# DefaultRui/VLN-VER

Hardware: AMD Instinct MI355X
Metric: viewpoints/sec (multi-view->voxel fwd+bwd), vocc.py config (higher is better)
Workload: dtype bf16

## Files before the change

include/ver_ops.h:

```cpp
#ifndef VER_OPS_H
#define VER_OPS_H

#include <stdint.h>

#ifdef __cplusplus
extern "C" {
#endif

#define VER_ABI_VERSION 31

#define VER_OK            0
#define VER_EINVAL       -1
#define VER_EUNSUPPORTED -2
#define VER_ELAUNCH      -3

#define VER_F32  0
#define VER_BF16 1

#define VER_I32  0
#define VER_I64  1

int         ver_abi_version(void);
const char* ver_last_error(void);

// ... 130 lines not shown
int ver_run_gather(const void* image, long image_stride, const int32_t* run_start, const int32_t* aug_idx,
                   void* rows, int B, int n_rows, int runs, int run_len, int n_aug, int row_elems, int dtype,
                   void* stream);
int ver_run_scatter(const void* rows, void* image, long image_stride, const int32_t* run_start, int B,
                    int n_rows, int runs, int run_len, int row_elems, int dtype, void* stream);

#define VER_OCC_MLP_CENTERED 2
long ver_occ_mlp_image_bytes(void);
int ver_occ_mlp_vector_floats(void);
int ver_occ_mlp_pack(const float* W1, const float* W2, const float* W3, void* image, void* stream);
int ver_occ_mlp_forward(const void* x, const void* image, const float* vectors, void* logits,
                        long N, int width, int classes, float eps, int flags, void* stream);
int ver_occ_mlp_forward_stats(const void* x, const void* image, const float* vectors, void* logits, float* rstd,
                              long N, int width, int classes, float eps, int flags, void* stream);
int ver_occ_mlp_backward(const void* x, const void* grad_logits, const void* image, const float* vectors,
                         void* grad_x, void* grad_a1, void* grad_a2, void* h1,
                         float* param_grads, long N, int width, int classes, float eps, int first_linear,
                         void* stream);
int ver_occ_mlp_backward_fused(const void* x, const void* grad_logits, const float* W2, const float* W3,
                               const float* vectors, void* grad_x, float* param_grads, long N, int width,
                               int classes, float eps, const float* grad_scale, int flags, void* stream);
int ver_occ_mlp_backward_fused_stats(const void* x, const void* grad_logits, const float* W2, const float* W3,
                                     const float* vectors, const float* rstd, void* grad_x, float* param_grads, long N,
                                     int width, int classes, float eps, const float* grad_scale, int flags, void* stream);
long ver_occ_mlp_backward_fused_slab_bytes(long N);
int ver_occ_mlp_backward_fused_slabs(const void* x, const void* grad_logits, const float* W2, const float* W3,
                                     const float* vectors, const float* rstd, void* grad_x, float* param_grads, float* slabs,
                                     long slab_bytes, long N, int width, int classes, float eps, const float* grad_scale,
                                     int flags, void* stream);

long ver_occ_predict_blocks(long N);
int  ver_occ_predict(const void* logits, int dtype, long N, int C, float threshold, int32_t* block_work,
                     int64_t* pairs, int64_t* count, void* stream);

int  ver_occ_confusion(const void* logits, int dtype, long rows_per_sample, int samples, int C, const uint8_t* labels,
                       const float* thresholds, int num_thresholds, int64_t* hist, void* stream);

int ver_occ_mlp_confusion(const void* x, const void* image, const float* vectors, const uint8_t* labels,
                          long rows_per_sample, int samples, const float* thresholds, int num_thresholds,
                          int64_t* hist, int width, int classes, float eps, int flags, void* stream);
int ver_occ_mlp_classes(const void* x, const void* image, const float* vectors, uint8_t* cls, float* prob,
                        long N, float threshold, int width, int classes, float eps, int flags, void* stream);

int  ver_wgrad_tn_splits(long M, int Ka, int N);
int  ver_wgrad_tn_splits_ld(long M, int Ka, int N, long ld);
long ver_wgrad_tn_workspace(long M, int Ka, int N, int splits);
int  ver_wgrad_tn(const void* a, long lda, const void* g, long ldg, long M, int Ka, int N, void* out, long ldo,
                  int out_dtype, int splits, int flags, void* workspace, long workspace_bytes, void* stream);
int  ver_wgrad_tn_segments(const void* lattice, int layout, int B, int H, int W, int C, const int* taps, int nseg, const void* cst,
                           int ncst, int cw, const void* g, long ldg, int N, void* out, long ldo, int out_dtype, int splits,
                           void* workspace, long workspace_bytes, void* stream);
int  ver_wgrad_tn_segments_splits(int B, int H, int W, long Ka, int N, long ldg);

int  ver_gemm_nn(const void* a, long lda, const void* w, long ldw, const float* bias, void* c, long ldc, long M, int K,
                 int N, int flags, void* stream);
int  ver_gemm_nn_taps(const void* lattice, int layout, int B, int H, int W, int C, const int* taps, int ntaps, const void* w,
                      long ldw, const float* rowpos, const float* bias, void* c, long ldc, int N, void* stream);
int  ver_gemm_nn_segments(const void* lattice, int layout, int B, int H, int W, int C, const int* taps, int ntaps,
                          const void* cst, int ncst, int cw, const void* w, long ldw, const float* rowpos, const float* bias,
                          void* c, long ldc, int N, void* stream);
int  ver_gemm_nn_planes(const void* lattice, int layout, int B, int H, int W, int C, long plane_elems, int nplanes,
                        const int* tap_plane, const int* taps, int ntaps, const void* cst, int ncst, int cw, const void* w,
                        long ldw, const float* rowpos, const float* bias, void* c, long ldc, int N, void* stream);
int  ver_gemm_nn_splits(long M, int K, int N);
int  ver_gemm_nn_splitk(const void* a, long lda, const void* w, long ldw, const float* bias, void* c, long ldc, long M, int K,
                        int N, int splits, void* workspace, long workspace_bytes, void* stream);

int ver_clip_adamw_step(void* const* table, const long* sizes, const int* chunk_tensor, const int* chunk_index,
                        int n_tensors, int n_chunks, int chunk_elems, float* partial, float* norm_out, float max_norm,
                        float lr, float beta1, float beta2, float eps, float weight_decay, long step, void* stream);

int ver_clip_adamw_step_tensors(void* const* table, const long* sizes, const int* chunk_tensor, const int* chunk_index,
                                const float* hyper, int* steps, int n_tensors, int n_chunks, int chunk_elems, float* partial,
                                float* norm_out, float max_norm, void* stream);

int ver_grad_pack(const void* const* table, const long* sizes, const long* offsets, const int* chunk_tensor,
                  const int* chunk_index, int n_tensors, int n_chunks, int chunk_elems, float scale, void* flat,
                  int flat_dtype, void* stream);

int ver_clip_adamw_step_flat(void* const* table, const long* sizes, const long* offsets, const int* chunk_tensor,
                             const int* chunk_index, const float* hyper, int* steps, const void* flat, int flat_dtype,
                             int n_tensors, int n_chunks, int chunk_elems, float* partial, float* norm_out, float max_norm,
                             void* stream);

int ver_lsa_solve(const float* cost, const int32_t* ncols, int32_t* match, int32_t* bad,
                  int P, int R, int Ccap, void* stream);

int ver_box3d_overlaps(const float* a, const int32_t* na, const float* b, const int32_t* nb, float* iou,
                       int S, int Acap, int Bcap, void* stream);

int ver_det_match(const float* pred_boxes, const int32_t* pred_labels, const float* pred_scores,
                  const uint8_t* pred_valid, const float* gt_boxes, const int32_t* gt_labels, const int32_t* ngt,
                  const float* thresholds, int num_thresholds, float* iou_max, int32_t* gt_index,
                  uint8_t* tp_bits, int64_t* npos, int num_classes, int S, int Pcap, int Gcap, void* stream);

int ver_det_costs(const void* cls, int cls_dtype, const float* box, int box_ld, const float* gt,
                  const int64_t* gt_labels, const int32_t* counts, float* cost, int L, int B, int Q, int C, int Gcap,
                  float w_cls, float alpha, float gamma, float eps, float w_reg, void* stream);
int ver_det_set_loss_forward(const void* cls, int cls_dtype, const float* box, int box_ld, const int32_t* match,
                             const float* gt, const int64_t* gt_labels, const int32_t* counts,
                             const float* code_weights, float* sums, int32_t* npos, int32_t* bad, int L, int B, int Q,
                             int C, int Gcap, float alpha, float gamma, void* stream);
int ver_det_set_loss_backward(const void* cls, int cls_dtype, const float* box, int box_ld, const int32_t* match,
                              const float* gt, const int64_t* gt_labels, const int32_t* counts,
                              const float* code_weights, const float* scale, void* grad_cls, float* grad_box, int L,
                              int B, int Q, int C, int Gcap, float alpha, float gamma, void* stream);
// ... 33 lines not shown
```

scratch/prof_summary.py:

```python
import sqlite3, sys, collections
def kernel_stats(path, out):
    db = sqlite3.connect(path); cur = db.cursor()
    rows = cur.execute("select name, count(*), sum(end-start), avg(end-start), min(end-start), max(end-start) from kernels group by name order by 3 desc").fetchall()
    tot = sum(r[2] for r in rows)
    with open(out, 'w') as f:
        f.write('# rocprofv3 --kernel-trace --stats summary (from %s)\n' % path.split('/')[-1])
        f.write('Name,Calls,TotalDurationNs,AverageNs,Percentage,MinNs,MaxNs\n')
        for r in rows:
            f.write('"%s",%d,%d,%.1f,%.2f,%d,%d\n' % (r[0].replace('"', "'")[:160], r[1], r[2], r[3], 100.0 * r[2] / tot, r[4], r[5]))
def pmc_stats(path, out, like=('k_sca', 'k_project', 'k_build', 'k_zero', 'k_msda', 'k_lattice', 'k_occ_mlp', 'k_focal')):
    db = sqlite3.connect(path); cur = db.cursor()
    rows = cur.execute("select kernel_name, counter_name, sum(value), count(distinct dispatch_id) from counters_collection group by kernel_name, counter_name").fetchall()
    with open(out, 'a') as f:
        f.write('# rocprofv3 --pmc per-dispatch averages (from %s)\n' % path.split('/')[-1])
        f.write('Kernel,Counter,PerDispatch,Dispatches\n')
        for k, c, v, n in sorted(rows):
            if any(l in k for l in like):
                f.write('"%s",%s,%.1f,%d\n' % (k.replace('(anonymous namespace)::', '').split('(')[0][:80], c, v / n, n))
def kernel_stats_timed(path, out, total_steps, skip_steps):
    db = sqlite3.connect(path); cur = db.cursor()
    rows = cur.execute("select name, start, end from kernels order by start").fetchall()
    per = collections.OrderedDict()
    for n, s, e in rows:
        per.setdefault(n, []).append(e - s)
    stats = []
    for n, d in per.items():
        c = len(d)
        if c % total_steps == 0 and c >= total_steps:
            k = c // total_steps
            d = d[skip_steps * k:]
            steps = total_steps - skip_steps
        else:
            steps = 0
        stats.append((n, len(d), sum(d), sum(d) / len(d), min(d), max(d), steps))
    stats.sort(key=lambda r: -r[2])
    tot = sum(r[2] for r in stats if r[6]) or 1
    with open(out, 'w') as f:
        f.write('# rocprofv3 --kernel-trace, dispatches of the TIMED steps only (%d of %d steps; from %s)\n' % (total_steps - skip_steps, total_steps, path.split('/')[-1]))
        f.write('Name,Calls,TotalDurationNs,AverageNs,PercentageOfTimedSteps,MinNs,MaxNs,Steps,NsPerStep\n')
        for n, c, t, a, lo, hi, st in stats:
            f.write('"%s",%d,%d,%.1f,%.2f,%d,%d,%d,%.0f\n' % (n.replace('"', "'")[:160], c, t, a, 100.0 * t / tot if st else 0.0, lo, hi, st, t / st if st else 0))
if __name__ == '__main__':
    if sys.argv[1] == 'kernels_timed':
        kernel_stats_timed(sys.argv[2], sys.argv[3], int(sys.argv[4]), int(sys.argv[5])); sys.exit(0)
    mode, path, out = sys.argv[1:4]
    (kernel_stats if mode == 'kernels' else pmc_stats)(path, out)
```

vln-ver_amd/csrc/build.py:

```python
import os
import subprocess
import sys
import tempfile

HERE = os.path.dirname(os.path.abspath(__file__))
PKG = os.path.dirname(HERE)
LIB = os.path.join(PKG, 'libver_hip.so')
SOURCES = ['ver_abi.hip', 'ver_msda.hip', 'ver_sca.hip', 'ver_lattice.hip', 'ver_mlp.hip', 'ver_loss.hip', 'ver_occ_mlp.hip', 'ver_layout.hip', 'ver_addln.hip', 'ver_post.hip', 'ver_wgrad.hip', 'ver_gemm.hip', 'ver_optim.hip', 'ver_assign.hip', 'ver_boxiou.hip', 'ver_setloss.hip', 'ver_decode.hip', 'ver_targets.hip', 'ver_dattn3d.hip', 'ver_mha.hip']
HEADERS = ['ver_common.h', 'ver_classify.h', 'ver_gemm_tile.h', os.path.join('..', '..', 'include', 'ver_ops.h')]
FLAGS = ['-O3', '-std=c++17', '--offload-arch=gfx950', '-fPIC', '-shared', '-munsafe-fp-atomics',
         '-Wall', '-Wno-unused-function']


TARGET_FEATURES = {'ver_occ_mlp.hip': ['-packed-fp32-ops']}
_HOST_PASS_NOISE = 'is not a recognized feature for this target'

OBJ_DIR = os.path.join(HERE, 'build')
CFLAGS = [f for f in FLAGS if f != '-shared']


def _newer(target, deps):
    if not os.path.exists(target):
        return True
    t = os.path.getmtime(target)
    return any(os.path.getmtime(d) > t for d in deps)


def stale():
    deps = [os.path.join(HERE, f) for f in SOURCES + HEADERS] + [os.path.abspath(__file__)]
    return _newer(LIB, deps)


ASAN_LIB = os.path.join(PKG, 'libver_hip_asan.so')
ASAN_FLAGS = ['-O1', '-g', '-fsanitize=address', '-fno-gpu-sanitize', '-shared-libsan', '-fno-omit-frame-pointer']


def asan_runtime():
    import glob
    hits = sorted(glob.glob('/opt/rocm/lib/llvm/lib/clang/*/lib/linux/libclang_rt.asan-x86_64.so'))
    return hits[-1] if hits else None


def build_hip(force=False, verbose=True, defines=(), lib=None, asan=False):
    if asan:
        lib = lib or ASAN_LIB
    lib = lib or LIB
    if not force and not defines and lib == LIB and not stale():
        return LIB
    if asan and not force and not _newer(lib, [os.path.join(HERE, f) for f in SOURCES + HEADERS] + [os.path.abspath(__file__)]):
        return lib
    hipcc = os.environ.get('HIPCC', '/opt/rocm/bin/hipcc')
    tag = ''.join('_' + d.replace('=', '-') for d in defines)
    os.makedirs(OBJ_DIR, exist_ok=True)
    hdrs = [os.path.join(HERE, h) for h in HEADERS] + [os.path.abspath(__file__)]
    objs, procs = [], []
    for src in SOURCES:
        path = os.path.join(HERE, src)
        mytag = tag if (defines and any(d.split('=')[0] in open(path).read() for d in defines)) else ''
        if asan:
            mytag += '_asan'
        obj = os.path.join(OBJ_DIR, src.replace('.hip', mytag + '.o'))
# ... 29 lines not shown
```

vln-ver_amd/csrc/ver_layout.hip:

```cpp
#include "ver_common.h"

namespace {
__device__ __forceinline__ uint16_t f32_to_bf16(float f) {
    const uint32_t u = __float_as_uint(f);
    if ((u & 0x7fffffffu) > 0x7f800000u) return (uint16_t)((u >> 16) | 0x40u);
    return (uint16_t)((u + 0x7fffu + ((u >> 16) & 1u)) >> 16);
}
constexpr int kTaps = 75;
constexpr int kPairs = 64;
}
#define VER_BLOCKS_VEC_SLICES 8

template <bool BF16>
__global__ __launch_bounds__(256) void k_convt_weight_fwd(const float* __restrict__ w, void* __restrict__ k, long P) {
    __shared__ float tile[kPairs * kTaps + 1];
    const long p0 = (long)blockIdx.x * kPairs;
    const int np = (int)((P - p0) < kPairs ? (P - p0) : kPairs);
    for (int i = threadIdx.x; i < np * kTaps; i += 256) tile[i] = w[p0 * kTaps + i];
    __syncthreads();
    for (int i = threadIdx.x; i < kTaps * kPairs; i += 256) {
        const int t = i / kPairs, p = i % kPairs;
        if (p >= np) continue;
        const int a = t / 25, b = (t / 5) % 5, c = t % 5;
        const float v = tile[p * kTaps + ((2 - a) * 5 + (4 - b)) * 5 + (4 - c)];
// ... 378 lines not shown
    }
}
__device__ __forceinline__ long row_map_piece(const RowMapLds& t, int period, int c, int piece_off) {
    const int4 ch = t.ch[c];
    int off = ch.z + piece_off, row = ch.y;
    while (off >= period) off -= period, ++row;
    const int sg = t.slot_seg[off >> 2];
    const int4 sp = t.seg[sg];
    return t.seg_base[sg] + (long)row * sp.z + ch.x * sp.y + (off - sp.x);
}
}

template <int LAYOUT, bool TO_ROWS, int CH>
__global__ __launch_bounds__(256) void k_lattice_rows(uint16_t* __restrict__ cl, uint16_t* __restrict__ rows, RowMap map,
                                                      int B, int Z, int H, int W, int C, int R) {
    extern __shared__ __attribute__((aligned(16))) unsigned char smem[];
    constexpr int VC = 8, VX = 4;
    const int P = R * W;
    const int ncb = (C + CH - 1) / CH;
    int r = (int)(blockIdx.x / ncb);
    const int hr = H / R;
    const int y0 = (r % hr) * R;
    r /= hr;
    const int z = r % Z;
    const int b = r / Z;
    const int c0 = (int)(blockIdx.x % ncb) * CH;
    const int nc = (C - c0) < CH ? (C - c0) : CH;
    const int ncv = nc / VC, npv = P / VX;
    unsigned* tile32 = reinterpret_cast<unsigned*>(smem);
    const int P2 = P >> 1, wp32 = (P2 + 2) & ~1;
    __shared__ RowMapLds lmap;
    row_map_setup(lmap, map, b, nc, (((long)c0 * Z + z) * H + y0) * W, (long)Z * H * W);
    if (TO_ROWS) {
        for (int i = threadIdx.x; i < P2 * ncv; i += 256) {
            const int p2 = i / ncv, cv = i - p2 * ncv;
            const int p = 2 * p2, yy = p / W, x = p - yy * W;
            const uint4 a = *reinterpret_cast<const uint4*>(cl + cl_index<LAYOUT>(b, z, y0 + yy, x, B, Z, H, W) * C + c0 + cv * VC);
            const uint4 q = *reinterpret_cast<const uint4*>(cl + cl_index<LAYOUT>(b, z, y0 + yy, x + 1, B, Z, H, W) * C + c0 + cv * VC);
            const unsigned aw[4] = {a.x, a.y, a.z, a.w}, qw[4] = {q.x, q.y, q.z, q.w};
            unsigned* dst = tile32 + (cv * VC) * wp32 + p2;
#pragma unroll
            for (int k = 0; k < 4; ++k) {
                dst[(2 * k) * wp32] = __builtin_amdgcn_perm(qw[k], aw[k], 0x05040100u);
                dst[(2 * k + 1) * wp32] = __builtin_amdgcn_perm(qw[k], aw[k], 0x07060302u);
            }
        }
        __syncthreads();
        for (int i = threadIdx.x; i < nc * npv; i += 256) {
            const int c = i / npv, pv = i - c * npv;
            const uint2 u = *reinterpret_cast<const uint2*>(tile32 + c * wp32 + 2 * pv);
            *reinterpret_cast<uint2*>(rows + row_map_piece(lmap, map.period, c, pv * VX)) = u;
        }
    } else {
        __syncthreads();
        for (int i = threadIdx.x; i < nc * npv; i += 256) {
            const int c = i / npv, pv = i - c * npv;
            *reinterpret_cast<uint2*>(tile32 + c * wp32 + 2 * pv) = *reinterpret_cast<const uint2*>(rows + row_map_piece(lmap, map.period, c, pv * VX));
        }
        __syncthreads();
        for (int i = threadIdx.x; i < P2 * ncv; i += 256) {
            const int p2 = i / ncv, cv = i - p2 * ncv;
            const int p = 2 * p2, yy = p / W, x = p - yy * W;
            const unsigned* srcw = tile32 + (cv * VC) * wp32 + p2;
            unsigned d[8];
#pragma unroll
            for (int j = 0; j < 8; ++j) d[j] = srcw[j * wp32];
            uint4 a, q;
            a.x = __builtin_amdgcn_perm(d[1], d[0], 0x05040100u); q.x = __builtin_amdgcn_perm(d[1], d[0], 0x07060302u);
            a.y = __builtin_amdgcn_perm(d[3], d[2], 0x05040100u); q.y = __builtin_amdgcn_perm(d[3], d[2], 0x07060302u);
            a.z = __builtin_amdgcn_perm(d[5], d[4], 0x05040100u); q.z = __builtin_amdgcn_perm(d[5], d[4], 0x07060302u);
            a.w = __builtin_amdgcn_perm(d[7], d[6], 0x05040100u); q.w = __builtin_amdgcn_perm(d[7], d[6], 0x07060302u);
            *reinterpret_cast<uint4*>(cl + cl_index<LAYOUT>(b, z, y0 + yy, x, B, Z, H, W) * C + c0 + cv * VC) = a;
            *reinterpret_cast<uint4*>(cl + cl_index<LAYOUT>(b, z, y0 + yy, x + 1, B, Z, H, W) * C + c0 + cv * VC) = q;
        }
    }
}

extern "C" int ver_convt_weight_forward(const float* weight, void* taps, long pairs, int dtype, void* stream) {
    VER_REQUIRE(pairs >= 0, VER_EINVAL, "ver_convt_weight_forward: negative size");
    VER_REQUIRE(dtype == VER_F32 || dtype == VER_BF16, VER_EINVAL, "ver_convt_weight_forward: dtype %d", dtype);
    if (pairs == 0) return VER_OK;
    VER_REQUIRE(weight && taps, VER_EINVAL, "ver_convt_weight_forward: null pointer argument");
    const unsigned blocks = (unsigned)((pairs + kPairs - 1) / kPairs);
    if (dtype == VER_BF16)
        hipLaunchKernelGGL(k_convt_weight_fwd<true>, dim3(blocks), dim3(256), 0, (hipStream_t)stream, weight, taps, pairs);
    else
        hipLaunchKernelGGL(k_convt_weight_fwd<false>, dim3(blocks), dim3(256), 0, (hipStream_t)stream, weight, taps, pairs);
    return ver_check_launch("ver_convt_weight_forward");
}

extern "C" int ver_convt_weight_backward(const void* grad_taps, float* grad_weight, long pairs, int dtype, void* stream) {
    VER_REQUIRE(pairs >= 0, VER_EINVAL, "ver_convt_weight_backward: negative size");
    VER_REQUIRE(dtype == VER_F32 || dtype == VER_BF16, VER_EINVAL, "ver_convt_weight_backward: dtype %d", dtype);
    if (pairs == 0) return VER_OK;
    VER_REQUIRE(grad_taps && grad_weight, VER_EINVAL, "ver_convt_weight_backward: null pointer argument");
    const unsigned blocks = (unsigned)((pairs + kPairs - 1) / kPairs);
    if (dtype == VER_BF16)
        hipLaunchKernelGGL(k_convt_weight_bwd<true>, dim3(blocks), dim3(256), 0, (hipStream_t)stream, grad_taps,
                           grad_weight, pairs);
    else
        hipLaunchKernelGGL(k_convt_weight_bwd<false>, dim3(blocks), dim3(256), 0, (hipStream_t)stream, grad_taps,
                           grad_weight, pairs);
    return ver_check_launch("ver_convt_weight_backward");
}

extern "C" int ver_convt_weight_backward_blocks(const void* blocks, const long* block_offsets, long ld, const void* prev_bias,
                                               const void* grad_v, float* grad_weight, int ci, int co, int dtype,
                                               void* stream) {
    VER_REQUIRE(ci >= 0 && co >= 0 && ld >= co, VER_EINVAL, "ver_convt_weight_backward_blocks: bad sizes (ci %d co %d ld %ld)",
                ci, co, ld);
    VER_REQUIRE(dtype == VER_F32 || dtype == VER_BF16, VER_EINVAL, "ver_convt_weight_backward_blocks: dtype %d", dtype);
    VER_REQUIRE((prev_bias == nullptr) == (grad_v == nullptr), VER_EINVAL,
                "ver_convt_weight_backward_blocks: prev_bias and grad_v come together");
    const long pairs = (long)ci * co;
    if (pairs == 0) return VER_OK;
    VER_REQUIRE(blocks && block_offsets && grad_weight, VER_EINVAL, "ver_convt_weight_backward_blocks: null pointer argument");
// ... 315 lines not shown
```

vln-ver_amd/dense_heads/row_linear.py:

```python
import torch
import torch.nn.functional as F

_CHUNK = 8000


class _RowLinear(torch.autograd.Function):

    @staticmethod
    def forward(ctx, x, weight, bias):
        w = weight.to(x.dtype)
        ctx.save_for_backward(x, w)
        ctx.has_bias = bias is not None
        ctx.weight_dtype = weight.dtype
        if bias is None:
            return x @ w.t()
        return torch.addmm(bias.to(x.dtype), x, w.t())

    @staticmethod
    def backward(ctx, g):
        x, w = ctx.saved_tensors
        g = g.contiguous()
        n, o = g.shape
        gx = g @ w if ctx.needs_input_grad[0] else None
        gb = None
        if ctx.has_bias:
            gb = g.sum(0, dtype=torch.float32)
        if g.dtype == torch.bfloat16 and x.dtype == torch.bfloat16 and n >= 4096 and min(o, x.shape[1]) >= 192:
            from ..hipops import wgrad_tn, wgrad_tn_supported
            if wgrad_tn_supported(g, x):
                wide = torch.float32 if ctx.weight_dtype == torch.float32 else torch.bfloat16
                if wide == torch.bfloat16 and gb is not None:
                    gb = gb.to(torch.bfloat16)
                return gx, wgrad_tn(g, x, out_dtype=wide), gb
        s = n // _CHUNK
        main = s * _CHUNK
        gw = x.new_zeros((o, x.shape[1]), dtype=torch.float32)
        if s:
            g3 = g[:main].view(s, _CHUNK, o)
            gw += torch.bmm(g3.transpose(1, 2), x[:main].view(s, _CHUNK, -1)).sum(0, dtype=torch.float32)
        if main < n:
            gw += (g[main:].t() @ x[main:]).float()
        return gx, gw, gb


def row_linear(x, weight, bias):
    if not x.is_cuda:
        return F.linear(x, weight, bias)
    if torch.is_autocast_enabled('cuda'):
        x = x.to(torch.get_autocast_dtype('cuda'))
    shape = x.shape
    with torch.autocast('cuda', enabled=False):
        y = _RowLinear.apply(x.reshape(-1, shape[-1]), weight, bias)
    return y.view(*shape[:-1], -1)
```

vln-ver_amd/hipops.py:

```python
import ctypes
import os
import re

import torch
from torch.autograd import Function
from torch.autograd.function import once_differentiable

_PKG = os.path.dirname(os.path.abspath(__file__))
LIB_PATH = os.environ.get('VER_HIP_LIB') or os.path.join(_PKG, 'libver_hip.so')
ABI_VERSION = 31
HEADER = os.path.join(os.path.dirname(_PKG), 'include', 'ver_ops.h')
_PARAMS = {'int': ctypes.c_int, 'long': ctypes.c_long, 'float': ctypes.c_float}
_RETURNS = {'int': ctypes.c_int, 'long': ctypes.c_long, 'const char*': ctypes.c_char_p}


class HipLibraryError(RuntimeError):
    pass


def prototypes(path=HEADER):
    if not os.path.exists(path):
        raise HipLibraryError('%s not found: the C ABI is bound from its prototypes' % path)
    text = re.sub(r'/\*.*?\*/|//[^\n]*|^\s*#[^\n]*', ' ', open(path).read(), flags=re.S | re.M)
    out = {}
# ... 288 lines not shown
        points = logits.shape[-1]
        gdt = lib().ver_sca_backward_grad_dtype(ctx.vdt, hd, points, map_h, map_w)
        gs = _gpu(grad_slots, 'grad_slots')
        gs_bf16 = gs.dtype == torch.bfloat16 and gdt == 1
        gs = gs.contiguous() if gs_bf16 else gs.float().contiguous()
        g_value = torch.empty((B, ncam, nk, heads, hd), dtype=torch.bfloat16 if gdt == 1 else torch.float32, device=value.device)
        g_off = torch.empty_like(offsets)
        g_log = torch.empty_like(logits)
        _launch('ver_sca_backward', lambda: lib().ver_sca_backward(
            _p(value), ctx.vdt, _p(offsets), _p(logits), _p(hit.uv), _p(hit.vis), _p(hit.vis_list),
            _p(hit.vis_cnt), _p(hit.fwd_list), _p(hit.fwd_cnt), _p(gs), _p(g_value), gdt, _p(g_off), _p(g_log), B, ncam,
            hit.Nq, hit.D, heads,
            hd, points, map_h, map_w, (2 if ctx.head_major else 0) | (4 if gs_bf16 else 0), _stream()),
            meta=dict(grad_slots_bf16=gs_bf16))
        g_value = g_value.to(value.dtype)
        if ctx.head_major:
            g_value = g_value.permute(3, 0, 1, 2, 4)
        return g_value, g_off, g_log, None, None, None, None, None, None


def sca_gather(value, offsets, logits, hit, map_h, map_w, prepared=None, head_major=False, lowp_out=False):
    return SCAGatherFunction.apply(value, offsets, logits, hit, map_h, map_w, prepared, head_major, lowp_out)


def sca_head_major_supported(dtype, head_dim, points, map_h, map_w):
    return dtype == torch.bfloat16 and bool(lib().ver_sca_head_major_supported(1, head_dim, points, map_h, map_w))


class HeadMajorLinearFunction(Function):

    @staticmethod
    def forward(ctx, x, weight, bias, heads):
        m, c_in = x.shape
        w = weight.to(x.dtype)
        hd = w.shape[0] // heads
        out = x.new_empty(heads, m, hd)
        b = bias.to(x.dtype).view(heads, hd)
        w3 = w.view(heads, hd, c_in)
        for h in range(heads):
            torch.addmm(b[h], x, w3[h].t(), out=out[h])
        ctx.save_for_backward(x, w)
        ctx.heads = heads
        return out

    @staticmethod
    @once_differentiable
    def backward(ctx, g):
        x, w = ctx.saved_tensors
        heads = ctx.heads
        m = x.shape[0]
        g2 = g.permute(1, 0, 2).reshape(m, -1)
        from .dense_heads.upsample import rows_tn
        dw = rows_tn(g2, x) if ctx.needs_input_grad[1] else None
        db = g2.sum(0, dtype=torch.float32) if ctx.needs_input_grad[2] else None
        dx = g2 @ w if ctx.needs_input_grad[0] else None
        return dx, dw, db, None


def head_major_linear(x, weight, bias, heads):
    return HeadMajorLinearFunction.apply(x, weight, bias, heads)


class LatticeIm2colFunction(Function):

    @staticmethod
    def forward(ctx, lattice, taps):
        lattice = _gpu(lattice, 'lattice')
        if lattice.dtype not in (torch.float32, torch.bfloat16):
            raise TypeError('lattice must be fp32 or bf16')
        B, Z, H, W, C = lattice.shape
        flat = [int(v) for t in taps for v in t]
        arr = (ctypes.c_int * len(flat))(*flat)
        dt = 1 if lattice.dtype == torch.bfloat16 else 0
        col = torch.empty(B * Z * H * W, len(taps) * C, dtype=lattice.dtype, device=lattice.device)
        _launch('ver_lattice_im2col', lambda: lib().ver_lattice_im2col(
            _p(lattice), _p(col), arr, len(taps), B, Z, H, W, C, dt, _stream()))
        ctx.geom = (B, Z, H, W, C, dt, arr, len(taps))
        return col

    @staticmethod
    @once_differentiable
    def backward(ctx, grad_col):
        B, Z, H, W, C, dt, arr, ntaps = ctx.geom
        want = torch.bfloat16 if dt else torch.float32
        g = _gpu(grad_col, 'grad_col').to(want).contiguous()
        grad = torch.empty(B, Z, H, W, C, dtype=want, device=g.device)
        _launch('ver_lattice_col2im', lambda: lib().ver_lattice_col2im(
            _p(g), _p(grad), arr, ntaps, B, Z, H, W, C, dt, _stream()))
        return grad, None


def lattice_im2col(lattice, taps):
    return LatticeIm2colFunction.apply(lattice, taps)


class ConvTWeightFunction(Function):

    @staticmethod
    def forward(ctx, weight, dtype):
        weight = _gpu(weight, 'weight')
        if weight.dtype != torch.float32 or tuple(weight.shape[2:]) != (3, 5, 5):
            raise TypeError('weight must be fp32 [Ci,Co,3,5,5]')
        if dtype not in (torch.float32, torch.bfloat16):
            raise TypeError('taps dtype must be fp32 or bf16')
        weight = weight.contiguous()
        ci, co = weight.shape[:2]
        taps = torch.empty(75, ci, co, dtype=dtype, device=weight.device)
# ... 1393 lines not shown
        invalid_offsets = idx(invalid_offsets, 'invalid_offsets', (bs + 1,))
        n_invalid = invalid.numel()
    total = bs * voxel_num
    padded = (total + 3) // 4 * 4
    if out is None:
        labels = torch.empty(padded, dtype=torch.uint8, device=dev)[:total]
        count = torch.empty(bs + 1, dtype=torch.int32, device=dev)
        bad = torch.empty(2, dtype=torch.int32, device=dev)
    else:
        labels, count, bad = out
        room = labels.untyped_storage().nbytes() - labels.storage_offset()
        if (labels.dtype != torch.uint8 or labels.numel() != total or not labels.is_contiguous() or labels.device != dev
                or room < padded):
            raise ValueError('%s: out labels must be %d contiguous uint8 on %s, allocated up to a multiple of 4 bytes' % (what, total, dev))
        labels = labels.view(-1)
        count, bad = idx(count, 'out count', (bs + 1,)), idx(bad, 'out bad', (2,))
    code = lambda t: 1 if t is not None and t.dtype == torch.int64 else 0
    _launch('ver_occ_targets', lambda: lib().ver_occ_targets(
        _p(pairs), code(pairs), _p(offsets), pairs.shape[0], _p(invalid), code(invalid), _p(invalid_offsets), n_invalid,
        _p(row_table), _p(labels), _p(count), _p(bad), voxel_num, zdim, classes, bs, _stream()))
    return labels, count, bad


def wgrad_tn_supported(a, g):
    return (a.is_cuda and g.is_cuda and a.dtype == torch.bfloat16 and g.dtype == torch.bfloat16 and a.dim() == 2
            and g.dim() == 2 and a.shape[0] == g.shape[0] and a.stride(1) == 1 and g.stride(1) == 1
            and a.stride(0) % 8 == 0 and g.stride(0) % 8 == 0 and a.data_ptr() % 16 == 0 and g.data_ptr() % 16 == 0
            and g.shape[1] % 4 == 0)


def wgrad_tn(a, g, out_dtype=None, splits=0, flags=0, out=None):
    if not wgrad_tn_supported(a, g):
        raise RuntimeError('wgrad_tn: unsupported operands %s %s / %s %s' % (tuple(a.shape), a.stride(), tuple(g.shape), g.stride()))
    m, ka = a.shape
    n = g.shape[1]
    out_dtype = out_dtype or a.dtype
    if out_dtype not in (torch.bfloat16, torch.float32):
        raise TypeError('wgrad_tn: out_dtype must be bf16 or fp32')
    L = lib()
    if splits <= 0:
        splits = L.ver_wgrad_tn_splits_ld(m, ka, n, max(a.stride(0), g.stride(0)))
    nbytes = L.ver_wgrad_tn_workspace(m, ka, n, splits)
    ws = torch.empty(nbytes // 4, dtype=torch.float32, device=a.device)
    if out is None:
        out = torch.empty(ka, n, dtype=out_dtype, device=a.device)
    elif not (out.is_cuda and out.shape == (ka, n) and out.dtype == out_dtype and out.stride(1) == 1):
        raise RuntimeError('wgrad_tn: out must be a [Ka, N] GPU matrix of out_dtype with unit column stride')
    _launch('ver_wgrad_tn', lambda: L.ver_wgrad_tn(
        _p(a), a.stride(0), _p(g), g.stride(0), m, ka, n, _p(out), out.stride(0), 1 if out_dtype == torch.bfloat16 else 0,
        splits, flags, _p(ws), nbytes, _stream()), meta=dict(flops=2.0 * m * ka * n))
    return out


def gemm_nn_supported(a, w):
    return (a.is_cuda and w.is_cuda and a.dtype == torch.bfloat16 and w.dtype == torch.bfloat16 and a.dim() == 2
            and w.dim() == 2 and a.shape[1] == w.shape[0] and a.stride(1) == 1 and w.stride(1) == 1
            and a.stride(0) % 8 == 0 and w.stride(0) % 8 == 0 and a.data_ptr() % 16 == 0 and w.data_ptr() % 16 == 0
            and a.shape[1] % 32 == 0 and a.shape[1] >= 64)


def gemm_nn_splits(m, k, n):
    return lib().ver_gemm_nn_splits(m, k, n)


def gemm_nn(a, w, bias=None, out=None, splits=None, timer_class='ver_gemm_nn'):
    if not gemm_nn_supported(a, w):
        raise RuntimeError('gemm_nn: unsupported operands %s %s / %s %s' % (tuple(a.shape), a.stride(), tuple(w.shape), w.stride()))
    m, k = a.shape
    n = w.shape[1]
    if out is None:
        out = torch.empty(m, n, dtype=torch.bfloat16, device=a.device)
    if out.shape != (m, n) or out.dtype != torch.bfloat16 or out.stride(1) != 1 or not out.is_cuda:
        raise RuntimeError('gemm_nn: out must be a bf16 [M, N] GPU matrix with unit column stride')
    if bias is not None:
        bias = _gpu(bias, 'bias').float().contiguous()
    if splits is None:
        splits = gemm_nn_splits(m, k, n)
    if splits > 1 and (n % 4 or out.stride(0) % 4 or out.data_ptr() % 8):
        splits = 1
    ws = torch.empty(splits * m * n, dtype=torch.float32, device=a.device) if splits > 1 else None
    _launch(timer_class, lambda: lib().ver_gemm_nn_splitk(
        _p(a), a.stride(0), _p(w), w.stride(0), _p(bias), _p(out), out.stride(0), m, k, n, splits, _p(ws),
        ws.numel() * 4 if ws is not None else 0, _stream()), meta=dict(flops=2.0 * m * k * n))
    return out


def gemm_nn_taps_supported(lattice, layout, w, c):
    return (lattice.is_cuda and lattice.dtype == torch.bfloat16 and lattice.is_contiguous() and layout in (PLAIN, ZSPLIT, PLANAR_ZSPLIT)
            and lattice.numel() * 2 < 2 ** 31 - 1 and c % 32 == 0 and c >= 64
            and (w is None or (w.is_cuda and w.dtype == torch.bfloat16 and w.dim() == 2 and w.stride(1) == 1 and w.stride(0) % 8 == 0
                               and w.data_ptr() % 16 == 0)))


def gemm_nn_taps(lattice, layout, combined_hw, taps, w, rowpos=None, bias=None, out=None, const_rows=None, planes=None,
                 timer_class='ver_gemm_nn'):
    lat, w = _gpu(lattice, 'lattice'), _gpu(w, 'w')
    plane_elems = nplanes = 0
    if planes is not None:
        nplanes, plane_elems = int(lat.shape[0]), int(lat[0].numel())
        if len(planes) != len(taps) or not lat.is_contiguous():
            raise ValueError('gemm_nn_taps: one source plane per tap, contiguous planes')
    lat_one = lat[0] if planes is not None else lat
    B, H, W, C, const_rows, ncst, cw, kdim, arr, ntaps = _segment_args(lat_one, layout, combined_hw, taps, const_rows, 'gemm_nn_taps')
    if not gemm_nn_taps_supported(lat_one, int(layout), w, C):
        raise RuntimeError('gemm_nn_taps: unsupported operands %s layout %d / %s %s' % (tuple(lat.shape), layout, tuple(w.shape), w.stride()))
    m, n = B * 2 * H * W, w.shape[1]
# ... 68 lines not shown
```

vln-ver_amd/modules/lowp_params.py:

```python
import contextlib
import functools

import torch
import torch.nn as nn

_ALIGN = 128


class _CastAll(torch.autograd.Function):

    @staticmethod
    def forward(ctx, offsets, total, *params):
        flat = torch.empty(total, dtype=torch.bfloat16, device=params[0].device)
        outs = [flat[o:o + p.numel()].view(p.shape) for o, p in zip(offsets, params)]
        torch._foreach_copy_(outs, [p.detach() for p in params])
        ctx.offsets, ctx.total = offsets, total
        ctx.set_materialize_grads(False)
        return tuple(outs)

    @staticmethod
    def backward(ctx, *grads):
        live = [i for i, g in enumerate(grads) if g is not None]
        out = [None] * len(grads)
        if live:
            flat = torch.empty(ctx.total, dtype=torch.float32, device=grads[live[0]].device)
            wide = [flat[ctx.offsets[i]:ctx.offsets[i] + grads[i].numel()].view(grads[i].shape) for i in live]
            torch._foreach_copy_(wide, [grads[i] for i in live])
            for i, w in zip(live, wide):
                out[i] = w
        return (None, None) + tuple(out)


class _LowpLinear(torch.autograd.Function):

    @staticmethod
    def forward(ctx, x, w, b):
        ctx.save_for_backward(x, w)
        ctx.has_bias = b is not None
        return x @ w.t() if b is None else torch.addmm(b, x, w.t())

    @staticmethod
    def backward(ctx, g):
        x, w = ctx.saved_tensors
        g = g.contiguous()
        gx = g @ w if ctx.needs_input_grad[0] else None
        gw = None
        if ctx.needs_input_grad[1]:
            from ..hipops import wgrad_tn, wgrad_tn_supported
            if g.shape[0] >= 512 and min(g.shape[1], x.shape[1]) >= 32 and wgrad_tn_supported(g, x):
                gw = wgrad_tn(g, x, out_dtype=torch.bfloat16)
            else:
                gw = g.t() @ x
        gb = g.sum(0) if (ctx.has_bias and ctx.needs_input_grad[2]) else None
        return gx, gw, gb


def _lent_linear_forward(mod, x):
    w, b = mod.weight, mod.bias
    x2 = x.reshape(-1, x.shape[-1])
    if x2.dtype != torch.bfloat16:
        x2 = x2.to(torch.bfloat16)
    with torch.autocast('cuda', enabled=False):
        y = _LowpLinear.apply(x2, w, b)
    return y.view(*x.shape[:-1], y.shape[-1])


class LowpParams:

    def __init__(self, roots):
        self.slots = []
        seen = set()
        for root in roots:
            for m in root.modules():
                if isinstance(m, nn.Linear):
                    names = ('weight', 'bias')
                elif isinstance(m, nn.MultiheadAttention):
                    names = ('in_proj_weight', 'in_proj_bias')
                else:
                    continue
                for n in names:
                    p = m._parameters.get(n)
                    if p is not None and id(p) not in seen and p.dtype == torch.float32:
                        seen.add(id(p))
                        self.slots.append((m, n))
        self.offsets, off = [], 0
        for m, n in self.slots:
            self.offsets.append(off)
            off += -(-m._parameters[n].numel() // _ALIGN) * _ALIGN
        self.total = off

    def applies(self, like):
        return (bool(self.slots) and like.is_cuda and torch.is_grad_enabled() and torch.is_autocast_enabled('cuda')
                and torch.get_autocast_dtype('cuda') == torch.bfloat16)

    @contextlib.contextmanager
    def lent(self):
        masters = [m._parameters[n] for m, n in self.slots]
        with torch.autocast('cuda', enabled=False):
            copies = _CastAll.apply(tuple(self.offsets), self.total, *masters)
        linears = {id(m): m for m, _ in self.slots if type(m) is nn.Linear}.values()
        try:
            for (m, n), c in zip(self.slots, copies):
                m._parameters[n] = c
            for m in linears:
                m.forward = functools.partial(_lent_linear_forward, m)
            yield
# ... 6 lines not shown
```

Baseline: 744.6.

## Add two-stage column-sum kernel for bias grads and rotate lattice tile columns

Adds a custom HIP column-sum kernel that reduces bf16 rows into fp32 partial sums across up to 1024 row groups, followed by a final reduction kernel. It replaces torch's g.sum(0) for bias gradients on large operands in three backward paths. Separately, the lattice layout kernel now rotates shared-memory tile columns per octet to avoid LDS bank conflicts, and unrolls its gather loads four-wide. The new reduction needs a workspace allocation and two launches, and its accumulation order differs from aten's.

Result: no change. 747.3 (median of 6 runs) (+0.4%).

```diff
diff --git a/include/ver_ops.h b/include/ver_ops.h
--- a/include/ver_ops.h
+++ b/include/ver_ops.h
@@ -206,6 +206,11 @@
                            void* workspace, long workspace_bytes, void* stream);
 int  ver_wgrad_tn_segments_splits(int B, int H, int W, long Ka, int N, long ldg);
 
+int  ver_colsum_groups(long M, int N);
+long ver_colsum_workspace(long M, int N);
+int  ver_colsum(const void* x, long ld, long M, int N, void* out, int out_dtype, void* workspace, long workspace_bytes,
+                void* stream);
+
 int  ver_gemm_nn(const void* a, long lda, const void* w, long ldw, const float* bias, void* c, long ldc, long M, int K,
                  int N, int flags, void* stream);
 int  ver_gemm_nn_taps(const void* lattice, int layout, int B, int H, int W, int C, const int* taps, int ntaps, const void* w,
diff --git a/scratch/colsum_bench.py b/scratch/colsum_bench.py
--- /dev/null
+++ b/scratch/colsum_bench.py
@@ -0,0 +1,69 @@
+import importlib
+import json
+import os
+import sys
+
+import torch
+
+ROOT = os.path.dirname(os.path.dirname(os.path.abspath(__file__)))
+sys.path.insert(0, ROOT)
+hip = importlib.import_module('vln-ver_amd.hipops')
+
+SWEEP_ROWS = (256, 512, 1024, 2048, 4096, 8192, 16384, 65536)
+SWEEP_COLS = (192, 768, 1536)
+STEP_SHAPES = ((225792, 768), (172800, 192), (172800, 768), (172800, 1536))
+
+
+def time_ms(fn, reps):
+    for _ in range(5):
+        fn()
+    torch.cuda.synchronize()
+    samples = []
+    for _ in range(3):
+        e0, e1 = torch.cuda.Event(enable_timing=True), torch.cuda.Event(enable_timing=True)
+        e0.record()
+        for _ in range(reps):
+            fn()
+        e1.record()
+        torch.cuda.synchronize()
+        samples.append(e0.elapsed_time(e1) / reps)
+    return sorted(samples)
+
+
+def main():
+    out = sys.argv[1]
+    reps = int(sys.argv[sys.argv.index('--reps') + 1]) if '--reps' in sys.argv else 50
+    dev = torch.device('cuda:0')
+    spoil = torch.empty(768 << 20, dtype=torch.uint8, device=dev)
+    with open(out, 'w') as f:
+        for m, n in [(m, n) for n in SWEEP_COLS for m in SWEEP_ROWS] + list(STEP_SHAPES):
+            g = torch.randn(m, n, device=dev).bfloat16()
+            big = m * n * 2 >= 32 << 20
+
+            def aten():
+                if big:
+                    spoil.zero_()
+                return g.sum(0)
+
+            def ours():
+                if big:
+                    spoil.zero_()
+                return hip.colsum(g)
+
+            base = time_ms(spoil.zero_, reps)[1] if big else 0.0
+            ta, to = time_ms(aten, reps), time_ms(ours, reps)
+            rec = dict(M=m, N=n, bytes=m * n * 2, aten_ms=[round(t - base, 5) for t in ta], colsum_ms=[round(t - base, 5) for t in to],
+                       cache_spoiler_ms=round(base, 5))
+            rec['speedup_median'] = round((ta[1] - base) / (to[1] - base), 3)
+            rec['colsum_TBps'] = round(m * n * 2 / ((to[1] - base) * 1e-3) / 1e12, 3)
+            rec['aten_TBps'] = round(m * n * 2 / ((ta[1] - base) * 1e-3) / 1e12, 3)
+            same = bool(torch.equal(hip.colsum(g), hip.colsum(g)))
+            err = float((hip.colsum(g, torch.float32).double() - g.double().sum(0)).abs().max())
+            rec.update(reproducible=same, max_abs_err_fp32=err)
+            f.write(json.dumps(rec) + '\n')
+            f.flush()
+            print(json.dumps(rec), flush=True)
+
+
+if __name__ == '__main__':
+    main()
diff --git a/scratch/lattice_rows_launch.py b/scratch/lattice_rows_launch.py
--- /dev/null
+++ b/scratch/lattice_rows_launch.py
@@ -0,0 +1,25 @@
+import importlib
+import os
+import sys
+
+import torch
+
+sys.path.insert(0, os.getcwd())
+hip = importlib.import_module('vln-ver_amd.hipops')
+ups = importlib.import_module('vln-ver_amd.dense_heads.upsample')
+opl = importlib.import_module('vln-ver_amd.dense_heads.occ_proj_lattice')
+B = int(sys.argv[1]) if len(sys.argv) > 1 else 192
+reps = int(sys.argv[2]) if len(sys.argv) > 2 else 3
+dev = torch.device('cuda:0')
+C, Z, Hl, Wl = 768, 4, 60, 60
+layout = ups.ZS_PLANAR_SPLIT
+plan = opl.get_plan(C, Z, 2 * Hl, 2 * Wl, dev)
+src = torch.randn(4, B, 2, Hl // 2, Wl // 2, 2, C, dtype=torch.bfloat16, device=dev)
+row_map, spans, total = opl._row_map_for(plan, B)
+buf = torch.zeros(total, dtype=torch.bfloat16, device=dev)
+got = torch.empty_like(src)
+for _ in range(reps):
+    hip.lattice_rows(src, buf, row_map, (Hl, Wl), layout, True)
+    hip.lattice_rows(got, buf, row_map, (Hl, Wl), layout, False)
+torch.cuda.synchronize()
+print('round trip equal:', bool(torch.equal(got, src)))
diff --git a/scratch/prof_summary.py b/scratch/prof_summary.py
--- a/scratch/prof_summary.py
+++ b/scratch/prof_summary.py
@@ -40,7 +40,26 @@
         f.write('Name,Calls,TotalDurationNs,AverageNs,PercentageOfTimedSteps,MinNs,MaxNs,Steps,NsPerStep\n')
         for n, c, t, a, lo, hi, st in stats:
             f.write('"%s",%d,%d,%.1f,%.2f,%d,%d,%d,%.0f\n' % (n.replace('"', "'")[:160], c, t, a, 100.0 * t / tot if st else 0.0, lo, hi, st, t / st if st else 0))
+def class_steps(path, out, total_steps, skip_steps, label, classes):
+    import json
+    db = sqlite3.connect(path); cur = db.cursor()
+    rows = cur.execute("select name, start, end from kernels order by start").fetchall()
+    with open(out, 'a') as f:
+        for cls in classes:
+            keys = cls.split('|')
+            d = [e - s for n, s, e in rows if any(k in n for k in keys)]
+            rec = dict(kind='class_steps', trace=label, kernels=keys, launches=len(d))
+            if d and len(d) % total_steps == 0:
+                k = len(d) // total_steps
+                steps = [sum(d[i * k:(i + 1) * k]) / 1e6 for i in range(skip_steps, total_steps)]
+                timed = d[skip_steps * k:]
+                rec.update(launches_per_step=k, ms_per_step=[round(v, 4) for v in steps], mean_ms=round(sum(steps) / len(steps), 4),
+                           spread_ms=round(max(steps) - min(steps), 4), launch_min_ms=round(min(timed) / 1e6, 4),
+                           launch_max_ms=round(max(timed) / 1e6, 4))
+            f.write(json.dumps(rec) + '\n')
 if __name__ == '__main__':
+    if sys.argv[1] == 'class_steps':
+        class_steps(sys.argv[2], sys.argv[3], int(sys.argv[4]), int(sys.argv[5]), sys.argv[6], sys.argv[7:]); sys.exit(0)
     if sys.argv[1] == 'kernels_timed':
         kernel_stats_timed(sys.argv[2], sys.argv[3], int(sys.argv[4]), int(sys.argv[5])); sys.exit(0)
     mode, path, out = sys.argv[1:4]
diff --git a/vln-ver_amd/csrc/build.py b/vln-ver_amd/csrc/build.py
--- a/vln-ver_amd/csrc/build.py
+++ b/vln-ver_amd/csrc/build.py
@@ -6,7 +6,7 @@
 HERE = os.path.dirname(os.path.abspath(__file__))
 PKG = os.path.dirname(HERE)
 LIB = os.path.join(PKG, 'libver_hip.so')
-SOURCES = ['ver_abi.hip', 'ver_msda.hip', 'ver_sca.hip', 'ver_lattice.hip', 'ver_mlp.hip', 'ver_loss.hip', 'ver_occ_mlp.hip', 'ver_layout.hip', 'ver_addln.hip', 'ver_post.hip', 'ver_wgrad.hip', 'ver_gemm.hip', 'ver_optim.hip', 'ver_assign.hip', 'ver_boxiou.hip', 'ver_setloss.hip', 'ver_decode.hip', 'ver_targets.hip', 'ver_dattn3d.hip', 'ver_mha.hip']
+SOURCES = ['ver_abi.hip', 'ver_msda.hip', 'ver_sca.hip', 'ver_lattice.hip', 'ver_mlp.hip', 'ver_loss.hip', 'ver_occ_mlp.hip', 'ver_layout.hip', 'ver_addln.hip', 'ver_post.hip', 'ver_wgrad.hip', 'ver_gemm.hip', 'ver_optim.hip', 'ver_assign.hip', 'ver_boxiou.hip', 'ver_setloss.hip', 'ver_decode.hip', 'ver_targets.hip', 'ver_dattn3d.hip', 'ver_mha.hip', 'ver_colsum.hip']
 HEADERS = ['ver_common.h', 'ver_classify.h', 'ver_gemm_tile.h', os.path.join('..', '..', 'include', 'ver_ops.h')]
 FLAGS = ['-O3', '-std=c++17', '--offload-arch=gfx950', '-fPIC', '-shared', '-munsafe-fp-atomics',
          '-Wall', '-Wno-unused-function']
diff --git a/vln-ver_amd/csrc/ver_colsum.hip b/vln-ver_amd/csrc/ver_colsum.hip
--- /dev/null
+++ b/vln-ver_amd/csrc/ver_colsum.hip
@@ -0,0 +1,127 @@
+#include "ver_common.h"
+
+namespace {
+constexpr int kColsumGroups = 1024;
+constexpr int kU = 8;
+constexpr int kFinalCols = 16, kFinalLanes = 16;
+
+__device__ __forceinline__ uint16_t colsum_bf16(float f) {
+    const uint32_t u = __float_as_uint(f);
+    if ((u & 0x7fffffffu) > 0x7f800000u) return (uint16_t)((u >> 16) | 0x40u);
+    return (uint16_t)((u + 0x7fffu + ((u >> 16) & 1u)) >> 16);
+}
+
+__device__ __forceinline__ void colsum_add(float (&acc)[8], const uint4 v) {
+    const uint32_t w[4] = {v.x, v.y, v.z, v.w};
+#pragma unroll
+    for (int k = 0; k < 4; ++k) {
+        acc[2 * k] += __uint_as_float(w[k] << 16);
+        acc[2 * k + 1] += __uint_as_float(w[k] & 0xffff0000u);
+    }
+}
+
+int colsum_row_lanes(int N) {
+    const int nv = N / 8;
+    return 256 / (nv < 256 ? nv : 256);
+}
+}
+
+__global__ __launch_bounds__(256) void k_colsum_part(const uint16_t* __restrict__ x, long ld, long M, int N, long rows_per,
+                                                     float* __restrict__ part) {
+    __shared__ __attribute__((aligned(16))) float red[256 * 8];
+    const int tid = threadIdx.x;
+    const int nv = N >> 3;
+    const int v0 = blockIdx.y * 256;
+    const int nvb = (nv - v0) < 256 ? (nv - v0) : 256;
+    const int RL = 256 / nvb;
+    const int rl = tid / nvb, cv = tid - rl * nvb;
+    const long r0 = (long)blockIdx.x * rows_per;
+    const long r1 = (r0 + rows_per) < M ? (r0 + rows_per) : M;
+    float acc[8] = {0.f, 0.f, 0.f, 0.f, 0.f, 0.f, 0.f, 0.f};
+    if (rl < RL) {
+        const uint16_t* p = x + (long)(v0 + cv) * 8;
+        for (long r = r0 + rl; r < r1; r += (long)kU * RL) {
+            uint4 v[kU];
+#pragma unroll
+            for (int u = 0; u < kU; ++u) {
+                const long row = r + (long)u * RL;
+                v[u] = row < r1 ? *reinterpret_cast<const uint4*>(p + row * ld) : make_uint4(0u, 0u, 0u, 0u);
+            }
+#pragma unroll
+            for (int u = 0; u < kU; ++u) colsum_add(acc, v[u]);
+        }
+    }
+    *reinterpret_cast<float4*>(red + tid * 8) = make_float4(acc[0], acc[1], acc[2], acc[3]);
+    *reinterpret_cast<float4*>(red + tid * 8 + 4) = make_float4(acc[4], acc[5], acc[6], acc[7]);
+    __syncthreads();
+    const int ncol = nvb * 8;
+    for (int c = tid; c < ncol; c += 256) {
+        float s = 0.f;
+        for (int q = 0; q < RL; ++q) s += red[q * ncol + c];
+        part[(long)blockIdx.x * N + v0 * 8 + c] = s;
+    }
+}
+
+template <bool BF16>
+__global__ __launch_bounds__(256) void k_colsum_final(const float* __restrict__ part, int G, int N, void* __restrict__ out) {
+    __shared__ float red[kFinalLanes][kFinalCols];
+    const int c = threadIdx.x & (kFinalCols - 1), q = threadIdx.x / kFinalCols;
+    const int col = blockIdx.x * kFinalCols + c;
+    float s = 0.f;
+    if (col < N) {
+#pragma unroll 8
+        for (int g = q; g < G; g += kFinalLanes) s += part[(long)g * N + col];
+    }
+    red[q][c] = s;
+    __syncthreads();
+    if (q == 0 && col < N) {
+        float t = red[0][c];
+#pragma unroll
+        for (int k = 1; k < kFinalLanes; ++k) t += red[k][c];
+        if (BF16)
+            reinterpret_cast<uint16_t*>(out)[col] = colsum_bf16(t);
+        else
+            reinterpret_cast<float*>(out)[col] = t;
+    }
+}
+
+extern "C" int ver_colsum_groups(long M, int N) {
+    if (M <= 0 || N < 8) return 0;
+    const long rows_min = (long)colsum_row_lanes(N) * kU;
+    const long g = (M + rows_min - 1) / rows_min;
+    return (int)(g < kColsumGroups ? g : kColsumGroups);
+}
+
+extern "C" long ver_colsum_workspace(long M, int N) { return (long)ver_colsum_groups(M, N) * (N > 0 ? N : 0) * 4; }
+
+extern "C" int ver_colsum(const void* x, long ld, long M, int N, void* out, int out_dtype, void* workspace,
+                          long workspace_bytes, void* stream) {
+    VER_REQUIRE(M >= 0 && N >= 0, VER_EINVAL, "ver_colsum: bad sizes (M %ld, N %d)", M, N);
+    VER_REQUIRE(ld >= N, VER_EINVAL, "ver_colsum: row pitch %ld below the %d columns", ld, N);
+    VER_REQUIRE(out_dtype == VER_F32 || out_dtype == VER_BF16, VER_EINVAL, "ver_colsum: out_dtype %d", out_dtype);
+    if (N == 0) return VER_OK;
+    VER_REQUIRE(out && (x || M == 0), VER_EINVAL, "ver_colsum: null pointer argument");
+    VER_REQUIRE(N % 8 == 0 && ld % 8 == 0 && ((uintptr_t)x & 15) == 0, VER_EUNSUPPORTED,
+                "ver_colsum: N and the row pitch must be multiples of 8 elements and x 16-byte aligned (16-byte loads)");
+    VER_REQUIRE(((uintptr_t)out & 3) == 0, VER_EINVAL, "ver_colsum: out is not aligned for its dtype");
+    const int G = ver_colsum_groups(M, N);
+    const long need = ver_colsum_workspace(M, N);
+    VER_REQUIRE(workspace_bytes >= need && (workspace || need == 0), VER_EINVAL,
+                "ver_colsum: workspace of %ld bytes, %ld needed (ver_colsum_workspace)", workspace_bytes, need);
+    VER_REQUIRE(((uintptr_t)workspace & 3) == 0, VER_EINVAL, "ver_colsum: workspace is not 4-byte aligned");
+    hipStream_t st = (hipStream_t)stream;
+    if (G > 0) {
+        const int RL = colsum_row_lanes(N);
+        long rows_per = (M + G - 1) / G;
+        rows_per = (rows_per + RL - 1) / RL * RL;
+        const dim3 grid((unsigned)G, (unsigned)((N / 8 + 255) / 256));
+        hipLaunchKernelGGL(k_colsum_part, grid, dim3(256), 0, st, (const uint16_t*)x, ld, M, N, rows_per, (float*)workspace);
+        if (int rc = ver_check_launch("ver_colsum")) return rc;
+    }
+    const dim3 fgrid((unsigned)((N + kFinalCols - 1) / kFinalCols));
+    if (out_dtype == VER_BF16)
+        hipLaunchKernelGGL(k_colsum_final<true>, fgrid, dim3(256), 0, st, (const float*)workspace, G, N, out);
+    else
+        hipLaunchKernelGGL(k_colsum_final<false>, fgrid, dim3(256), 0, st, (const float*)workspace, G, N, out);
+    return ver_check_launch("ver_colsum");
+}
diff --git a/vln-ver_amd/csrc/ver_layout.hip b/vln-ver_amd/csrc/ver_layout.hip
--- a/vln-ver_amd/csrc/ver_layout.hip
+++ b/vln-ver_amd/csrc/ver_layout.hip
@@ -454,16 +454,41 @@
             *reinterpret_cast<uint2*>(rows + row_map_piece(lmap, map.period, c, pv * VX)) = u;
         }
     } else {
+        auto rot = [&](int octet) {
+            int s = 2 * octet;
+            while (s >= wp32) s -= wp32;
+            return s;
+        };
         __syncthreads();
-        for (int i = threadIdx.x; i < nc * npv; i += 256) {
-            const int c = i / npv, pv = i - c * npv;
-            *reinterpret_cast<uint2*>(tile32 + c * wp32 + 2 * pv) = *reinterpret_cast<const uint2*>(rows + row_map_piece(lmap, map.period, c, pv * VX));
+        constexpr int kU = 4;
+        const int n_pieces = nc * npv;
+        for (int i0 = threadIdx.x; i0 < n_pieces; i0 += 256 * kU) {
+            uint2 v[kU];
+            int at[kU];
+#pragma unroll
+            for (int u = 0; u < kU; ++u) {
+                const int i = i0 + u * 256;
+                at[u] = -1;
+                v[u] = make_uint2(0u, 0u);
+                if (i < n_pieces) {
+                    const int c = i / npv, pv = i - c * npv;
+                    v[u] = *reinterpret_cast<const uint2*>(rows + row_map_piece(lmap, map.period, c, pv * VX));
+                    int col = 2 * pv + rot(c >> 3);
+                    if (col >= wp32) col -= wp32;
+                    at[u] = c * wp32 + col;
+                }
+            }
+#pragma unroll
+            for (int u = 0; u < kU; ++u)
+                if (at[u] >= 0) *reinterpret_cast<uint2*>(tile32 + at[u]) = v[u];
         }
         __syncthreads();
         for (int i = threadIdx.x; i < P2 * ncv; i += 256) {
             const int p2 = i / ncv, cv = i - p2 * ncv;
             const int p = 2 * p2, yy = p / W, x = p - yy * W;
-            const unsigned* srcw = tile32 + (cv * VC) * wp32 + p2;
+            int col = p2 + rot(cv);
+            if (col >= wp32) col -= wp32;
+            const unsigned* srcw = tile32 + (cv * VC) * wp32 + col;
             unsigned d[8];
 #pragma unroll
             for (int j = 0; j < 8; ++j) d[j] = srcw[j * wp32];
diff --git a/vln-ver_amd/dense_heads/row_linear.py b/vln-ver_amd/dense_heads/row_linear.py
--- a/vln-ver_amd/dense_heads/row_linear.py
+++ b/vln-ver_amd/dense_heads/row_linear.py
@@ -24,7 +24,8 @@
         gx = g @ w if ctx.needs_input_grad[0] else None
         gb = None
         if ctx.has_bias:
-            gb = g.sum(0, dtype=torch.float32)
+            from ..hipops import bias_grad
+            gb = bias_grad(g, torch.float32)
         if g.dtype == torch.bfloat16 and x.dtype == torch.bfloat16 and n >= 4096 and min(o, x.shape[1]) >= 192:
             from ..hipops import wgrad_tn, wgrad_tn_supported
             if wgrad_tn_supported(g, x):
diff --git a/vln-ver_amd/hipops.py b/vln-ver_amd/hipops.py
--- a/vln-ver_amd/hipops.py
+++ b/vln-ver_amd/hipops.py
@@ -364,7 +364,7 @@
         g2 = g.permute(1, 0, 2).reshape(m, -1)
         from .dense_heads.upsample import rows_tn
         dw = rows_tn(g2, x) if ctx.needs_input_grad[1] else None
-        db = g2.sum(0, dtype=torch.float32) if ctx.needs_input_grad[2] else None
+        db = bias_grad(g2, torch.float32) if ctx.needs_input_grad[2] else None
         dx = g2 @ w if ctx.needs_input_grad[0] else None
         return dx, dw, db, None
 
@@ -1864,6 +1864,37 @@
     return out
 
 
+def colsum_supported(x):
+    return (x.is_cuda and x.dtype == torch.bfloat16 and x.dim() == 2 and x.shape[1] > 0 and x.shape[1] % 8 == 0
+            and x.stride(1) == 1 and x.stride(0) >= x.shape[1] and x.stride(0) % 8 == 0 and x.data_ptr() % 16 == 0)
+
+
+def colsum(x, out_dtype=None):
+    if not colsum_supported(x):
+        raise RuntimeError('colsum: unsupported operand %s %s %s' % (tuple(x.shape), x.stride(), x.dtype))
+    out_dtype = out_dtype or x.dtype
+    if out_dtype not in (torch.bfloat16, torch.float32):
+        raise TypeError('colsum: out_dtype must be bf16 or fp32')
+    m, n = x.shape
+    L = lib()
+    nbytes = L.ver_colsum_workspace(m, n)
+    ws = torch.empty(nbytes // 4, dtype=torch.float32, device=x.device)
+    out = torch.empty(n, dtype=out_dtype, device=x.device)
+    _launch('ver_colsum', lambda: L.ver_colsum(_p(x), x.stride(0), m, n, _p(out), 1 if out_dtype == torch.bfloat16 else 0,
+                                               _p(ws), nbytes, _stream()))
+    return out
+
+
+COLSUM_MIN_ELEMS = 1 << 21
+
+
+def bias_grad(g, out_dtype=None):
+    if (g.dim() == 2 and g.shape[0] * g.shape[1] >= COLSUM_MIN_ELEMS and out_dtype in (None, torch.bfloat16, torch.float32)
+            and colsum_supported(g)):
+        return colsum(g, out_dtype)
+    return g.sum(0) if out_dtype is None else g.sum(0, dtype=out_dtype)
+
+
 def gemm_nn_supported(a, w):
     return (a.is_cuda and w.is_cuda and a.dtype == torch.bfloat16 and w.dtype == torch.bfloat16 and a.dim() == 2
             and w.dim() == 2 and a.shape[1] == w.shape[0] and a.stride(1) == 1 and w.stride(1) == 1
diff --git a/vln-ver_amd/modules/lowp_params.py b/vln-ver_amd/modules/lowp_params.py
--- a/vln-ver_amd/modules/lowp_params.py
+++ b/vln-ver_amd/modules/lowp_params.py
@@ -51,7 +51,10 @@
                 gw = wgrad_tn(g, x, out_dtype=torch.bfloat16)
             else:
                 gw = g.t() @ x
-        gb = g.sum(0) if (ctx.has_bias and ctx.needs_input_grad[2]) else None
+        gb = None
+        if ctx.has_bias and ctx.needs_input_grad[2]:
+            from ..hipops import bias_grad
+            gb = bias_grad(g)
         return gx, gw, gb
 
 
```
